# SunBangjie/FYP-BidirectionalPathTracer

Hardware: AMD Instinct MI355X
Metric: Mrays/s + RMSE vs the scalar oracle, BDPT pass, Sponza-class scene 1920x1080 depth 8 (higher is better)
Workload: dtype f32

## Files before the change

fyp-bidirectionalpathtracer_amd/csrc/api.cpp:

```cpp
#include <hip/hip_runtime.h>

#include <cmath>
#include <cstdio>
#include <cstdlib>
#include <cstring>
#include <future>
#include <functional>
#include <atomic>
#include <chrono>
#include <string>
#include <thread>
#include <vector>

#include "../../include/bdpt.h"
#include <new>

#include "bvh.h"
#include "kernels.h"
#include "refit.h"
#include "scene_bvh.h"

using namespace bdpt;

namespace {
// ... 8 lines not shown

struct bdpt_ctx {
  int device = 0;
  int numCUs = 256;
  std::string err;
  bool haveScene = false, haveCamera = false, haveSize = false;
  SceneDev S{};
  std::vector<void*> sceneAllocs;
  bdpt_bvh_info bvhInfo{};
  bdpt_camera cam{};
  bdpt_environment env{};
  uint32_t W = 0, H = 0, maxDepth = 0;
  std::vector<std::pair<uint32_t, uint32_t>> rowRanges;
  uint32_t tileRows = 0;
  SplatLayout sl{1, 1, 0};
  bdpt_stripes stripes{0, 1, 0};
  PathBuf P{};
  std::vector<void*> frameAllocs;
  unsigned long long* splat = nullptr;
  unsigned long long* ownSplat = nullptr;
  DevCounters* counters = nullptr;
  hipStream_t lastStream = nullptr;
  bool timing = false;
  hipEvent_t ev[kMaxStages + 1]{};
  const char* stageNames[kMaxStages]{};
  int numStages = 0;
  bool evCreated = false;
  static constexpr int kMaxSideStages = 4;
  hipEvent_t sideEv[2 * kMaxSideStages]{};
  const char* sideNames[kMaxSideStages]{};
  int numSideStages = 0;
  int lazyRounds = 3;
  LaunchGrids grids{};
  int* stackOvf = nullptr;
  uint32_t stackOvfStride = 0;
  unsigned long long* rayCursor = nullptr;
  unsigned long long* adaptiveSum = nullptr;
  bdpt_gbuffer ownGb{};
  float4* bmfrPos[2] = {nullptr, nullptr};
  float4* bmfrNorm[2] = {nullptr, nullptr};
  float4* bmfrNoisy[2] = {nullptr, nullptr};
  float4* bmfrFiltered[2] = {nullptr, nullptr};
  uint8_t* bmfrAccept = nullptr;
  uint32_t* bmfrPrevPixel = nullptr;
  int bmfrRead = 0;
  hipStream_t walkStream = nullptr;
  hipEvent_t evFork = nullptr, evJoin = nullptr, evSplat = nullptr;
  uint32_t* hintPix = nullptr;
  bool hints = true;
  bdpt_camera hintCam{};
  bool hintCamValid = false;
  uint32_t numVertices = 0, numTriangles = 0;
  uint32_t* lightMaps = nullptr;
  bool refitReady = false;
  BvhRefitPlan refitPlan;
  RefitDev refit{};
  uint32_t numUpdates = 0;
  float* stage[3] = {nullptr, nullptr, nullptr};
  void* pinned = nullptr;
  size_t pinnedBytes = 0;
  hipEvent_t evStage = nullptr, evOrder = nullptr;
  bool stageInFlight = false;
  unsigned long long* groupSplat = nullptr;
  uint8_t* groupLightIdx = nullptr;
};

namespace {

template <class F>
void hostParallelFor(size_t n, const F& f) {
  const int threads = bvhBuildThreads();
  if (threads <= 1 || n < 65536) {
    f((size_t)0, n);
    return;
  }
  WorkerScope pool;
  const size_t chunk = (n + (size_t)threads - 1) / (size_t)threads;
  for (int t = 1; t < threads; t++) {
    const size_t a = std::min(n, chunk * (size_t)t), b = std::min(n, a + chunk);
    if (a < b) pool.spawn([&f, a, b] { f(a, b); });
  }
  f((size_t)0, std::min(n, chunk));
  pool.join();
}

bool fail(bdpt_ctx* c, const std::string& m) {
  if (c) c->err = m;
  return false;
}
#define HIPCHK(ctx, expr)                                                                       \
  do {                                                                                          \
    hipError_t e_ = (expr);                                                                     \
    if (e_ != hipSuccess) {                                                                     \
      fail(ctx, std::string(#expr) + ": " + hipGetErrorString(e_));                             \
      return BDPT_E_HIP;                                                                        \
    }                                                                                           \
  } while (0)

template <class T>
int devAlloc(bdpt_ctx* c, std::vector<void*>& pool, T** out, size_t count) {
  void* p = nullptr;
  size_t bytes = std::max<size_t>(count * sizeof(T), 16);
  hipError_t e = hipMalloc(&p, bytes);
  if (e != hipSuccess) {
    fail(c, std::string("hipMalloc(") + std::to_string(bytes) + "): " + hipGetErrorString(e));
    return BDPT_E_NOMEM;
  }
  pool.push_back(p);
  *out = reinterpret_cast<T*>(p);
  return BDPT_OK;
}
template <class T>
int devUpload(bdpt_ctx* c, std::vector<void*>& pool, const T** out, const T* host, size_t count) {
  T* d = nullptr;
  int rc = devAlloc(c, pool, &d, count);
  if (rc) return rc;
  if (count) {
    std::string e;
    if (!bvhUploadStaged(d, host, count * sizeof(T), e)) {
      fail(c, e);
      return BDPT_E_HIP;
    }
  }
  *out = d;
  return BDPT_OK;
}
void freePool(std::vector<void*>& pool) {
  for (void* p : pool) (void)hipFree(p);
  pool.clear();
}
void freeLightGroups(bdpt_ctx* c) {
  if (c->groupSplat) (void)hipFree(c->groupSplat);
  if (c->groupLightIdx) (void)hipFree(c->groupLightIdx);
  c->groupSplat = nullptr;
  c->groupLightIdx = nullptr;
}

#define ENTER(ctx) HIPCHK(ctx, hipSetDevice((ctx)->device))

bool streamIsCapturing(hipStream_t st) {
  hipStreamCaptureStatus cs = hipStreamCaptureStatusNone;
  if (hipStreamIsCapturing(st, &cs) != hipSuccess) return false;
  return cs != hipStreamCaptureStatusNone;
}

int allocOwnGbuffer(bdpt_ctx* c) {
  if (c->ownGb.worldPosition) return BDPT_OK;
  const size_t n = (size_t)c->W * c->H;
  const size_t mark = c->frameAllocs.size();
  bdpt_gbuffer g{};
  int rc;
  if ((rc = devAlloc(c, c->frameAllocs, &g.worldPosition, n * 4)) || (rc = devAlloc(c, c->frameAllocs, &g.worldNormal, n * 4)) ||
      (rc = devAlloc(c, c->frameAllocs, &g.materialDiffuse, n * 4)) || (rc = devAlloc(c, c->frameAllocs, &g.materialSpecRough, n * 4)) ||
      (rc = devAlloc(c, c->frameAllocs, &g.materialExtraParams, n * 4)) || (rc = devAlloc(c, c->frameAllocs, &g.emissive, n * 4))) {
    while (c->frameAllocs.size() > mark) {
      (void)hipFree(c->frameAllocs.back());
      c->frameAllocs.pop_back();
    }
    return rc;
  }
  c->ownGb = g;
  return BDPT_OK;
}

int allocBmfrHistory(bdpt_ctx* c) {
  if (c->bmfrAccept) return BDPT_OK;
// ... 252 lines not shown
    std::future<SideUploads>& f;
    ~SideJoin() {
      if (!f.valid()) return;
      try {
        SideUploads u = f.get();
        for (void* q : u.pool) (void)hipFree(q);
      } catch (...) {
      }
    }
  } sideJoin{side};
  SceneBvh sb;
  try {
    std::string treeError;
    struct Build {
      BvhDeviceBuild* b;
      ~Build() { bvhDeviceBuildEnd(b); }
    } build{bvhDeviceBuildBegin(c->device, std::getenv("BDPT_HOST_COLLAPSE") == nullptr)};
    buildSceneBvh(d, 0, -1.0f, -1.0f, std::getenv("BDPT_NO_ALPHA_CLASSIFY") == nullptr, sb, buildBinaryTreeOnDevice, build.b, &treeError, packOnDevice, makeReferencesOnDevice,
                  std::getenv("BDPT_HOST_COLLAPSE") == nullptr, std::getenv("BDPT_HOST_PRIORITIES") == nullptr);
    if (sb.bvh.deviceRecs) c->sceneAllocs.push_back(sb.bvh.deviceRecs);
    if (!treeError.empty()) {
      fail(c, "scene: " + treeError);
      return treeError.find("2^31") != std::string::npos ? BDPT_E_LIMIT : (treeError.find("out of device memory") != std::string::npos ? BDPT_E_NOMEM : BDPT_E_HIP);
    }
  } catch (const std::bad_alloc&) {
    fail(c, "scene: out of host memory while building the acceleration structure");
    return BDPT_E_NOMEM;
  }
  lap("buildSceneBvh");
  Bvh& bvh = sb.bvh;
  const std::vector<uint32_t>& alphaTris = sb.alphaTris;
  if (bvh.maxStack > (uint32_t)kBvhMaxStack) {
    fail(c, "bvh needs a deeper traversal stack than the device provides");
    return BDPT_E_LIMIT;
  }
  if (!bvh.deviceRecs && !bvh.recs.empty()) {
    const BvhRec* dRecs = nullptr;
    if (int rc0 = devUpload(c, c->sceneAllocs, &dRecs, bvh.recs.data(), bvh.recs.size())) return rc0;
    bvh.deviceRecs = const_cast<BvhRec*>(dRecs);
    bvh.deviceNumRecs = bvh.recs.size();
  }
  if (!bvh.deviceRecs) {
    fail(c, "scene: the acceleration structure has no records");
    return BDPT_E_HIP;
  }
  c->bvhInfo.numNodes = bvh.numNodes;
  c->bvhInfo.numTriangles = d->numTriangles;
  c->bvhInfo.maxDepth = bvh.maxDepth;
  c->bvhInfo.nodeBytes = sizeof(BvhRec);
  c->bvhInfo.triBytes = sizeof(BvhTri);
  c->bvhInfo.sahCost = bvh.sahCost;
  c->bvhInfo.maxStack = bvh.maxStack;
  c->bvhInfo.numReferences = bvh.numRefs;
  c->bvhInfo.numDropped = bvh.numDropped;
  c->bvhInfo.numAlphaMode = sb.numAlphaMode;
  c->bvhInfo.numAlwaysPass = sb.numAlwaysPass;

  int rc;
  {
    SideUploads u = side.get();
    c->sceneAllocs.insert(c->sceneAllocs.end(), u.pool.begin(), u.pool.end());
    if (u.err != hipSuccess) {
      fail(c, std::string("scene upload: ") + (u.what.empty() ? std::string(hipGetErrorString(u.err)) : u.what));
      return u.err == hipErrorOutOfMemory ? BDPT_E_NOMEM : BDPT_E_HIP;
    }
    c->S.shade = reinterpret_cast<const float4*>(u.shade);
    c->S.indices = u.indices;
    if (d->bitangents) {
      c->S.bitangents = u.bitangents;
      c->S.hasBitangents = 1;
    }
  }
  lap("shading records + uploads (joined)");
  c->S.recs = reinterpret_cast<const uint4*>(bvh.deviceRecs);
  c->S.numRecs = (uint32_t)bvh.deviceNumRecs;
  if ((rc = devUpload(c, c->sceneAllocs, &c->S.materials, d->materials, d->numMaterials))) return rc;
  std::vector<TexDev> texs(d->numTextures);
  for (uint32_t i = 0; i < d->numTextures; i++) {
    const bdpt_texture& t = d->textures[i];
    if (!t.rgba8 || !t.width || !t.height) {
      fail(c, "scene: empty texture");
      return BDPT_E_INVALID;
    }
    const uint8_t* px;
    if ((rc = devUpload(c, c->sceneAllocs, &px, t.rgba8, (size_t)t.width * t.height * 4))) return rc;
    texs[i] = TexDev{px, t.width, t.height, t.srgb, 0};
  }
  if ((rc = devUpload(c, c->sceneAllocs, &c->S.textures, texs.data(), texs.size()))) return rc;
  {
    std::vector<TexDev> matTex((size_t)d->numMaterials * 4, TexDev{nullptr, 0, 0, 0, 0});
    for (uint32_t mi = 0; mi < d->numMaterials; mi++) {
      const bdpt_material& mm = d->materials[mi];
      const int ids[4] = {mm.texBaseColor, mm.texSpecular, mm.texEmissive, mm.texNormal};
      for (int k = 0; k < 4; k++)
        if (ids[k] >= 0) matTex[(size_t)mi * 4 + k] = texs[(size_t)ids[k]];
    }
    if ((rc = devUpload(c, c->sceneAllocs, &c->S.matTex, matTex.data(), matTex.size()))) return rc;
  }
  {
    float4* dAlpha = nullptr;
    if ((rc = devAlloc(c, c->sceneAllocs, &dAlpha, std::max<size_t>(alphaTris.size(), 1) * 4))) return rc;
    if (alphaTris.empty()) {
      HIPCHK(c, hipMemset(dAlpha, 0, 4 * sizeof(float4)));
    } else {
      const uint32_t* dList = nullptr;
      std::vector<void*> scratch;
      if ((rc = devUpload(c, scratch, &dList, alphaTris.data(), alphaTris.size()))) {
        freePool(scratch);
        return rc;
      }
      launchAlphaRecs(c->S, dList, (uint32_t)alphaTris.size(), dAlpha, nullptr);
      const hipError_t e = hipDeviceSynchronize();
      freePool(scratch);
      HIPCHK(c, e);
    }
    c->S.alphaRecs = dAlpha;
  }
  lap("indices, textures, alpha");
  SceneConst sc;
  std::memset(&sc, 0, sizeof(sc));
  std::memcpy(sc.lights, d->lights, sizeof(bdpt_light) * d->numLights);
  for (int i = 0; i < 256; i++) {
    double cc = (double)i / 255.0;
    double l = (cc <= 0.04045) ? cc / 12.92 : std::pow((cc + 0.055) / 1.055, 2.4);
    sc.srgbLut[i] = (float)l;
  }
  if ((rc = devUpload(c, c->sceneAllocs, &c->S.sc, &sc, 1))) return rc;
  c->S.numLights = d->numLights;
  c->hints = std::getenv("BDPT_NO_HINTS") == nullptr;
  if (c->hints) {
    uint32_t res = 512;
    if (const char* e = std::getenv("BDPT_LIGHT_MAP_RES")) res = (uint32_t)std::max(0, std::min(2048, std::atoi(e)));
    if (res) {
      uint32_t* maps = nullptr;
      if ((rc = devAlloc(c, c->sceneAllocs, &maps, (size_t)6 * res * res * d->numLights))) return rc;
      launchLightMaps(c->S, maps, res, nullptr);
      HIPCHK(c, hipDeviceSynchronize());
      c->S.lightMap = maps;
      c->S.lightMapRes = res;
      c->lightMaps = maps;
    }
  }
  if (c->hintPix) HIPCHK(c, hipMemset(c->hintPix, 0xFF, (size_t)c->W * c->H * sizeof(uint32_t)));
  c->hintCamValid = false;
  lap("light maps");
  c->numVertices = d->numVertices;
  c->numTriangles = d->numTriangles;
  c->haveScene = true;
  return BDPT_OK;
}
int bdpt_set_scene(bdpt_ctx* c, const bdpt_scene_desc* d) {
  try {
    return setSceneImpl(c, d);
  } catch (const std::bad_alloc&) {
    fail(c, "scene: out of host memory while building the acceleration structure");
    return BDPT_E_NOMEM;
  } catch (const std::exception& e) {
    fail(c, std::string("scene: ") + e.what());
    return BDPT_E_INVALID;
  }
}


int bdpt_get_bvh_info(const bdpt_ctx* c, bdpt_bvh_info* out) {
  if (!c || !out) return BDPT_E_INVALID;
  if (!c->haveScene) return BDPT_E_STATE;
  *out = c->bvhInfo;
  return BDPT_OK;
}

int bdpt_set_camera(bdpt_ctx* c, const bdpt_camera* cam) {
  if (!c || !cam) return BDPT_E_INVALID;
  c->cam = *cam;
  c->haveCamera = true;
  return BDPT_OK;
}

int bdpt_set_environment(bdpt_ctx* c, const bdpt_environment* env) {
  if (!c) return BDPT_E_INVALID;
  if (env && env->envMap && (!env->width || !env->height)) {
    fail(c, "environment: a map needs a width and a height");
    return BDPT_E_INVALID;
  }
  c->env = env ? *env : bdpt_environment{};
  if (!c->env.envMap) c->env.width = c->env.height = 0;
  return BDPT_OK;
}

namespace {
int ensureRefit(bdpt_ctx* c, hipStream_t st) {
  if (c->refitReady) return BDPT_OK;
  if (streamIsCapturing(st)) {
    fail(c, "update: the first update needs bdpt_prepare(BDPT_PREPARE_REFIT) before stream capture");
    return BDPT_E_STATE;
// ... 1252 lines not shown
```

fyp-bidirectionalpathtracer_amd/csrc/device_scene.hpp:

```cpp
#pragma once
#include "device_math.hpp"
#include "kernels.h"

namespace bdpt {
#define BD __device__ __forceinline__

struct f4 {
  float x, y, z, w;
};
BD f4 lerp4(f4 a, f4 b, float s) {
  return f4{a.x + (b.x - a.x) * s, a.y + (b.y - a.y) * s, a.z + (b.z - a.z) * s, a.w + (b.w - a.w) * s};
}
BD int wrapi(int i, int n) {
  int m = i % n;
  return (m < 0) ? m + n : m;
}
BD f4 texel(const SceneDev& S, const TexDev& t, int ix, int iy) {
  const uchar4 p = *reinterpret_cast<const uchar4*>(t.px + ((size_t)iy * t.w + (size_t)ix) * 4);
  f4 r;
  if (t.srgb) {
    r.x = S.sc->srgbLut[p.x];
    r.y = S.sc->srgbLut[p.y];
    r.z = S.sc->srgbLut[p.z];
  } else {
    r.x = (float)p.x / 255.0f;
    r.y = (float)p.y / 255.0f;
    r.z = (float)p.z / 255.0f;
  }
  r.w = (float)p.w / 255.0f;
  return r;
}
BD f4 sampleBilinearT(const SceneDev& S, const TexDev& t, float u, float v) {
  float x = u * (float)t.w - 0.5f;
  float y = v * (float)t.h - 0.5f;
  float x0 = floorf(x), y0 = floorf(y);
  float fx = x - x0, fy = y - y0;
  int ix0 = wrapi((int)x0, (int)t.w), iy0 = wrapi((int)y0, (int)t.h);
  int ix1 = wrapi(ix0 + 1, (int)t.w), iy1 = wrapi(iy0 + 1, (int)t.h);
  f4 t00 = texel(S, t, ix0, iy0), t10 = texel(S, t, ix1, iy0);
  f4 t01 = texel(S, t, ix0, iy1), t11 = texel(S, t, ix1, iy1);
  return lerp4(lerp4(t00, t10, fx), lerp4(t01, t11, fx), fy);
}
BD f4 sampleBilinear(const SceneDev& S, int texId, float u, float v) { return sampleBilinearT(S, S.textures[texId], u, v); }
BD f4 sampleTexture(const SceneDev& S, int texId, float u, float v, f4 factor, uint32_t mode) {
  if (mode == BDPT_CHANNEL_UNUSED) return f4{0, 0, 0, 0};
  if (mode == BDPT_CHANNEL_CONST || texId < 0) return factor;
  return sampleBilinear(S, texId, u, v);
}
BD f4 sampleTextureT(const SceneDev& S, const TexDev& t, int texId, float u, float v, f4 factor, uint32_t mode) {
  if (mode == BDPT_CHANNEL_UNUSED) return f4{0, 0, 0, 0};
  if (mode == BDPT_CHANNEL_CONST || texId < 0) return factor;
  return sampleBilinearT(S, t, u, v);
}

struct MatDev {
  f4 baseColor, specular;
  f3 emissive;
  float alphaThreshold, IoR;
  uint32_t flags;
  int texBase, texSpec, texEmis, texNorm;
};
BD MatDev loadMaterial(const SceneDev& S, uint32_t id) {
  const float4* m = reinterpret_cast<const float4*>(S.materials + id);
  float4 a = m[0], b = m[1], c = m[2], d = m[3];
  MatDev r;
  r.baseColor = f4{a.x, a.y, a.z, a.w};
  r.specular = f4{b.x, b.y, b.z, b.w};
  r.emissive = mk(c.x, c.y, c.z);
  r.alphaThreshold = c.w;
  r.IoR = d.x;
  r.flags = __float_as_uint(d.y);
  uint32_t t0 = __float_as_uint(d.z), t1 = __float_as_uint(d.w);
  r.texBase = (int)(int16_t)(t0 & 0xffffu);
  r.texSpec = (int)(int16_t)(t0 >> 16);
  r.texEmis = (int)(int16_t)(t1 & 0xffffu);
  r.texNorm = (int)(int16_t)(t1 >> 16);
  return r;
}

BD bool alphaTestFails(const SceneDev& S, uint32_t rec, float bu, float bv) {
  const float4* r = S.alphaRecs + (size_t)rec * 4;
  const float4 a0 = r[0], a1 = r[1], a2 = r[2], a3 = r[3];
  const uint32_t mode = __float_as_uint(a2.x);
  float alpha = 0.0f;
  if (mode == 1u) {
    alpha = a1.w;
  } else if (mode == 2u) {
    float u = 0, v = 0;
    const float b0 = 1.0f - bu - bv;
    u += a0.x * b0;
    v += a0.y * b0;
    u += a0.z * bu;
    v += a0.w * bu;
    u += a1.x * bv;
    v += a1.y * bv;
    const int tw = (int)__float_as_uint(a2.y), th = (int)__float_as_uint(a2.z);
    const uint8_t* px = reinterpret_cast<const uint8_t*>(((unsigned long long)__float_as_uint(a3.y) << 32) | (unsigned long long)__float_as_uint(a3.x));
    const float x = u * (float)tw - 0.5f, y = v * (float)th - 0.5f;
    const float x0 = floorf(x), y0 = floorf(y);
    const float fx = x - x0, fy = y - y0;
    const int ix0 = wrapi((int)x0, tw), iy0 = wrapi((int)y0, th);
    const int ix1 = wrapi(ix0 + 1, tw), iy1 = wrapi(iy0 + 1, th);
    const float t00 = (float)px[((size_t)iy0 * tw + (size_t)ix0) * 4 + 3] / 255.0f, t10 = (float)px[((size_t)iy0 * tw + (size_t)ix1) * 4 + 3] / 255.0f;
    const float t01 = (float)px[((size_t)iy1 * tw + (size_t)ix0) * 4 + 3] / 255.0f, t11 = (float)px[((size_t)iy1 * tw + (size_t)ix1) * 4 + 3] / 255.0f;
    const float top = t00 + (t10 - t00) * fx, bot = t01 + (t11 - t01) * fx;
    alpha = top + (bot - top) * fy;
  }
  return alpha < a1.z;
}

struct AlphaIn {
  float4 a0, a1, a2, a3;
};
BD void alphaTexels(const AlphaIn& r, float bu, float bv, bool run, float& fx, float& fy, float& t00, float& t10, float& t01, float& t11) {
  fx = fy = t00 = t10 = t01 = t11 = 0.0f;
  if (!run || __float_as_uint(r.a2.x) != 2u) return;
  float u = 0, v = 0;
  const float b0 = 1.0f - bu - bv;
  u += r.a0.x * b0;
  v += r.a0.y * b0;
  u += r.a0.z * bu;
  v += r.a0.w * bu;
  u += r.a1.x * bv;
  v += r.a1.y * bv;
  const int tw = (int)__float_as_uint(r.a2.y), th = (int)__float_as_uint(r.a2.z);
  const uint8_t* px = reinterpret_cast<const uint8_t*>(((unsigned long long)__float_as_uint(r.a3.y) << 32) | (unsigned long long)__float_as_uint(r.a3.x));
  const float x = u * (float)tw - 0.5f, y = v * (float)th - 0.5f;
  const float x0 = floorf(x), y0 = floorf(y);
  fx = x - x0;
  fy = y - y0;
  const int ix0 = wrapi((int)x0, tw), iy0 = wrapi((int)y0, th);
  const int ix1 = wrapi(ix0 + 1, tw), iy1 = wrapi(iy0 + 1, th);
  t00 = (float)px[((size_t)iy0 * tw + (size_t)ix0) * 4 + 3];
  t10 = (float)px[((size_t)iy0 * tw + (size_t)ix1) * 4 + 3];
  t01 = (float)px[((size_t)iy1 * tw + (size_t)ix0) * 4 + 3];
  t11 = (float)px[((size_t)iy1 * tw + (size_t)ix1) * 4 + 3];
}
BD bool alphaVerdict(const AlphaIn& r, float fx, float fy, float t00, float t10, float t01, float t11) {
  const uint32_t mode = __float_as_uint(r.a2.x);
  float alpha = 0.0f;
  if (mode == 1u) {
    alpha = r.a1.w;
  } else if (mode == 2u) {
    const float w00 = t00 / 255.0f, w10 = t10 / 255.0f, w01 = t01 / 255.0f, w11 = t11 / 255.0f;
    const float top = w00 + (w10 - w00) * fx, bot = w01 + (w11 - w01) * fx;
    alpha = top + (bot - top) * fy;
  }
  return alpha < r.a1.z;
}
BD void alphaTestFails2(const SceneDev& S, bool need0, uint32_t rec0, float u0, float v0, bool need1, uint32_t rec1, float u1, float v1,
                        bool& fail0, bool& fail1) {
  AlphaIn r0, r1;
  r0.a0 = r0.a1 = r0.a2 = r0.a3 = r1.a0 = r1.a1 = r1.a2 = r1.a3 = make_float4(0.0f, 0.0f, 0.0f, 0.0f);
  if (need0) {
    const float4* p = S.alphaRecs + (size_t)rec0 * 4;
    r0.a0 = p[0];
    r0.a1 = p[1];
    r0.a2 = p[2];
    r0.a3 = p[3];
  }
  if (need1) {
    const float4* p = S.alphaRecs + (size_t)rec1 * 4;
    r1.a0 = p[0];
    r1.a1 = p[1];
    r1.a2 = p[2];
    r1.a3 = p[3];
  }
  float fx0, fy0, a00, a10, a01, a11, fx1, fy1, b00, b10, b01, b11;
  alphaTexels(r0, u0, v0, need0, fx0, fy0, a00, a10, a01, a11);
  alphaTexels(r1, u1, v1, need1, fx1, fy1, b00, b10, b01, b11);
  fail0 = need0 && alphaVerdict(r0, fx0, fy0, a00, a10, a01, a11);
  fail1 = need1 && alphaVerdict(r1, fx1, fy1, b00, b10, b01, b11);
}

struct Shading {
  f3 posW, V, N, diffuse, specular, emissive;
  float opacity, linearRoughness, roughness, IoR;
};
template <bool NMAP>
BD Shading shadeHit(const SceneDev& S, uint32_t prim, float bu, float bv, f3 camPosW) {
  const float4* r = S.shade + (size_t)prim * kShadeRecF4;
  const float4 r0 = r[0], r1 = r[1], r2 = r[2], r3 = r[3], r4 = r[4], r5 = r[5], r6 = r[6];
  const float b0 = 1.0f - bu - bv;
  float u = 0, v = 0;
  f3 normalW = mk(0), posW = mk(0);
  u += r1.z * b0;
  v += r1.w * b0;
  normalW = normalW + mk(r0.w, r1.x, r1.y) * b0;
  posW = posW + mk(r0.x, r0.y, r0.z) * b0;
  u += r3.z * bu;
  v += r3.w * bu;
  normalW = normalW + mk(r2.w, r3.x, r3.y) * bu;
  posW = posW + mk(r2.x, r2.y, r2.z) * bu;
  u += r5.z * bv;
  v += r5.w * bv;
  normalW = normalW + mk(r4.w, r5.x, r5.y) * bv;
  posW = posW + mk(r4.x, r4.y, r4.z) * bv;
  normalW = normalize(normalW);

  const uint32_t matId = __float_as_uint(r6.x);
  const MatDev m = loadMaterial(S, matId);
  const TexDev tBase = S.matTex[(size_t)matId * 4], tSpec = S.matTex[(size_t)matId * 4 + 1], tEmis = S.matTex[(size_t)matId * 4 + 2];
  Shading sd;
  f4 base = sampleTextureT(S, tBase, m.texBase, u, v, m.baseColor, BDPT_FLAG_DIFFUSE_TYPE(m.flags));
  sd.opacity = m.baseColor.w;
  sd.posW = posW;
  sd.V = normalize(camPosW - posW);
  sd.N = normalize(normalW);
  f4 spec = sampleTextureT(S, tSpec, m.texSpec, u, v, m.specular, BDPT_FLAG_SPECULAR_TYPE(m.flags));
  f3 baseRgb = mk(base.x, base.y, base.z);
  if (BDPT_FLAG_SHADING_MODEL(m.flags) == BDPT_SHADING_MODEL_METAL_ROUGH) {
    sd.diffuse = lerp3(baseRgb, mk(0), spec.z);
    sd.specular = lerp3(mk(0.04f), baseRgb, spec.z);
    sd.linearRoughness = spec.y;
  } else {
    sd.diffuse = baseRgb;
    sd.specular = mk(spec.x, spec.y, spec.z);
    sd.linearRoughness = 1.0f - spec.w;
  }
// ... 40 lines not shown
```

fyp-bidirectionalpathtracer_amd/csrc/kernels.h:

```cpp
#pragma once
#include <hip/hip_runtime.h>
#include <stdint.h>

#include "../../include/bdpt.h"

namespace bdpt {

constexpr int kWave = 64;
#ifndef KSTACK
#define KSTACK 32
#endif
constexpr int kStackEntries = KSTACK;
#ifndef BDPT_STACK_LDS
#define BDPT_STACK_LDS 24
#endif
constexpr int kStackLds = BDPT_STACK_LDS < KSTACK ? BDPT_STACK_LDS : KSTACK;
constexpr int kMaxPersistentPerCU = 32;
constexpr int kStackOvfRows = KSTACK - kStackLds;
constexpr int kShadeRecF4 = 7;
constexpr uint32_t kNoRay = 0xFFFFFFFFu;
constexpr uint32_t kNumSubQueues = 32;
#ifndef BDPT_FETCH_CHUNK
#define BDPT_FETCH_CHUNK 256
#endif
constexpr uint32_t kFetchChunk = BDPT_FETCH_CHUNK;
constexpr uint32_t kCursorStride = 32;
constexpr uint32_t kCursorBlock = kNumSubQueues * kCursorStride;
#ifndef BDPT_RAY_SUBQUEUES
#define BDPT_RAY_SUBQUEUES 32
#endif
constexpr uint32_t kNumRaySubQueues = BDPT_RAY_SUBQUEUES;
constexpr uint32_t kRayCursorBlock = kNumRaySubQueues * kCursorStride;
constexpr uint32_t kCounterShards = 64;

enum : int { F_COL = 0, F_POS = 3, F_N = 6, F_V = 9, F_DIF = 12, F_SPEC = 15, F_ROUGH = 18, F_ISSPEC = 19, F_PDF = 20, NF = 21 };
constexpr int NF4 = 6;
enum : int { PATH_EYE = 0, PATH_LIGHT = 1 };
enum : int { RAY_TERMS = 0, RAY_PAIRS = 1 };

struct TexDev {
  const uint8_t* px;
  uint32_t w, h, srgb, pad;
};

struct SceneConst {
  bdpt_light lights[BDPT_MAX_LIGHTS];
  float srgbLut[256];
};

struct SceneDev {
  const uint4* recs;
  const float4* shade;
  const float* bitangents;
  const uint32_t* indices;
  const bdpt_material* materials;
  const TexDev* textures;
  const TexDev* matTex;
  const SceneConst* sc;
  uint32_t numLights;
  uint32_t hasBitangents;
  uint32_t numRecs;
  const float4* alphaRecs;
  int* stackOvf;
  uint32_t stackOvfStride;
  const uint32_t* lightMap;
  uint32_t lightMapRes;
};

struct DevCounters {
  unsigned long long v[kCounterShards][32];
};
enum : int {
  C_RAYS_PRIMARY = 0, C_RAYS_EYE, C_RAYS_LIGHT, C_RAYS_NEE, C_RAYS_SPLAT, C_RAYS_CONNECT,
  C_NODE_CLOSEST, C_TRI_CLOSEST, C_NODE_SHADOW, C_TRI_SHADOW, C_PIX_VALID, C_SPLATS, C_RAYS_LAZY,
  C_STACK_MAX,
  C_ALPHA_CLOSEST, C_ALPHA_SHADOW,
  C_HINT_NEE, C_HINT_SPLAT
};

inline __host__ __device__ uint32_t numConnectPairs(uint32_t D) {
  uint32_t n = 0;
  for (uint32_t t = 2; t <= D; t++) n += (t < D - 1) ? t : (D - 1);
  return n;
}

struct PathBuf {
  float* v;
  float* rayDir;
  const uint32_t* pix;
  uint32_t* seedE;
  uint32_t* seedL;
  uint8_t* eyeLast;
  uint8_t* lightLast;
  uint8_t* lightReal;
  uint32_t* queue[3];
  uint32_t pathSubCap;
  uint32_t* qcount;
  uint32_t* qhead;
  float* rayQ;
  float* rayContrib;
  uint8_t* rayVis;
  uint32_t* rayCount;
  uint32_t* rayHead;
  uint32_t raySubCap[2];
  uint32_t rayBase[2];
  uint32_t* slotRay;
  uint32_t* splatPix;
  float* misE;
  float* misL;
  uint8_t* lazyCursor;
  uint32_t* lazyRay;
  uint32_t* lazyCount;
  uint32_t rayCap;
  uint32_t Np, D1;
};

struct SplatLayout {
  uint32_t stripeRows, owners, chunkRows;
};
inline __host__ __device__ size_t splatIndex(const SplatLayout& L, uint32_t W, uint32_t x, uint32_t y) {
  const uint32_t s = y / L.stripeRows;
  const uint32_t owner = s % L.owners, row = (s / L.owners) * L.stripeRows + (y - s * L.stripeRows);
  return ((size_t)owner * L.chunkRows + row) * W + x;
}

struct FrameDev {
  bdpt_camera cam;
  bdpt_params p;
  uint32_t W, H;
  SplatLayout sl;
  float* out;
  unsigned long long* splat;
  bdpt_gbuffer gb;
  DevCounters* counters;
  const float* envMap;
  uint32_t envW, envH;
  float envColor[3];
  const uint32_t* hintPix;
};

struct GroupDev {
  float* planes;
  unsigned long long* splat;
  uint8_t* lightIdx;
  uint32_t numLights;
  uint64_t framePix;
};

struct MaskDev {
  const uint8_t* mask;
  uint32_t* eye;
  uint32_t* eyeCount;
  const uint32_t* walkEye;
  const uint32_t* walkEyeCount;
};

enum class FrameKind { Plain, Groups, Masked };
struct FrameVariant {
  FrameKind kind = FrameKind::Plain;
  GroupDev groups{};
  MaskDev mask{};
};

struct GBufferDev {
  bdpt_camera cam;
  bdpt_gbuffer_params gp;
  uint32_t W, H, Np;
  const uint32_t* pix;
  bdpt_gbuffer gb;
  DevCounters* counters;
  uint32_t* hintPix;
};

struct BmfrDev {
  uint32_t W, H, frame;
  uint32_t full, doPre;
  float m[16];
  const float4* curPos;
  const uint16_t* curNorm;
  const uint16_t* albedo;
  float4* noisy;
  const float4 *prevPosR, *prevNormR, *prevNoisyR, *prevFilteredR;
  float4 *prevPosW, *prevNormW, *prevNoisyW, *prevFilteredW;
  uint8_t* accept;
  uint32_t* prevPixel;
};
void launchBmfr(const BmfrDev& A, uint32_t flags, hipStream_t st);

void launchGBuffer(const SceneDev& S, const GBufferDev& G, hipStream_t st);
void launchAlphaRecs(const SceneDev& S, const uint32_t* alphaTris, uint32_t n, float4* out, hipStream_t st);
void launchHintFill(const SceneDev& S, const GBufferDev& G, hipStream_t st);
void launchLightMaps(const SceneDev& S, uint32_t* maps, uint32_t res, hipStream_t st);
void launchInitPaths(const SceneDev& S, const FrameDev& F, const PathBuf& P, const FrameVariant& V, hipStream_t st);
struct LaunchGrids {
  uint32_t walk[16] = {};
  uint32_t shadow[2] = {0, 0};
  uint32_t rays[3] = {0, 0, 0};
};
void launchWalk(const SceneDev& S, const FrameDev& F, const PathBuf& P, const FrameVariant& V, LaunchGrids& G, int numCUs,
                hipStream_t st);
void launchMisPrefix(const FrameDev& F, const PathBuf& P, hipStream_t st);
void launchGenNee(const SceneDev& S, const FrameDev& F, const PathBuf& P, hipStream_t st);
void launchGenSplat(const SceneDev& S, const FrameDev& F, const PathBuf& P, hipStream_t st);
void launchGenConnect(const SceneDev& S, const FrameDev& F, const PathBuf& P, hipStream_t st);
void launchTraceShadow(const SceneDev& S, const FrameDev& F, const PathBuf& P, int rayClass, LaunchGrids& G, int numCUs, hipStream_t st);
void launchTraceRays(const SceneDev& S, const float4* rays, uint32_t cap, const uint32_t* count, unsigned long long* cursor, int mode,
                     float4* hits, uint8_t* vis, LaunchGrids& G, int numCUs, hipStream_t st);
void launchGather(const FrameDev& F, const PathBuf& P, const FrameVariant& V, uint32_t* lazyList, uint32_t* lazyCount, hipStream_t st);
void launchLazyGen(const FrameDev& F, const PathBuf& P, const uint32_t* list, const uint32_t* listCount, int batch, hipStream_t st);
void launchLazyCheck(const FrameDev& F, const PathBuf& P, const FrameVariant& V, const uint32_t* list, const uint32_t* listCount,
                     int batch, uint32_t* nextList, uint32_t* nextCount, hipStream_t st);
constexpr int kLazyBatchDiv = 8;
constexpr int kMaxLazyRounds = 8;
void launchResolve(const unsigned long long* splat, bool tileLocal, uint32_t splatRow0, const SplatLayout& L, float* out, uint32_t W,
                   const uint32_t* pix, uint32_t Np, hipStream_t st);
void launchFrameResolve(const FrameDev& F, const PathBuf& P, const FrameVariant& V, hipStream_t st);
struct AdaptiveDev {
  float4* mean;
  float* m2;
  uint32_t* count;
  uint8_t* mask;
  uint32_t* active;
  float4* frame;
  uint32_t W, H;
  float threshold, epsilon;
  uint32_t minSamples, maxSamples, blockSize;
};
void launchAdaptiveUpdate(const AdaptiveDev& A, unsigned long long* scratch, hipStream_t st);
void launchAdaptiveReset(const AdaptiveDev& A, hipStream_t st);
void launchAccumulate(float* last, float* cur, uint32_t accumCount, uint32_t maxAccum, uint64_t numTexels, hipStream_t st);
void launchAccumulateTile(float* last, float* cur, uint32_t accumCount, uint32_t maxAccum, const uint32_t* pix, uint32_t Np,
                          hipStream_t st);
void launchTilePack(const void* frame, void* packed, uint32_t bytesPerPixel, const uint32_t* pix, uint32_t Np, hipStream_t st);
void launchTileUnpack(const void* packed, void* frame, uint32_t bytesPerPixel, uint32_t W, uint32_t H, uint32_t stripeRows, uint32_t owners,
                      uint32_t owner, uint32_t packedRows, hipStream_t st);
void launchTestRng(const uint32_t* v0, const uint32_t* v1, uint32_t n, uint32_t draws, uint32_t* states, float* floats,
                   hipStream_t st);
void launchTestTrace(const SceneDev& S, const float* rays, uint32_t n, int mode, int32_t* prim, float* tuv, hipStream_t st);
void launchTestTraceShadow(const SceneDev& S, const float* planes, uint32_t cap, const uint32_t* count, uint32_t* head, uint8_t* vis,
                           DevCounters* counters, float tmin, int numCUs, hipStream_t st);
void launchTestBsdf(const float* in, uint32_t n, uint32_t matIndex, float* out, hipStream_t st);

}
```

fyp-bidirectionalpathtracer_amd/csrc/kernels.hip:

```cpp
#include "kernels.h"

#include <algorithm>
#include <type_traits>

#include "device_math.hpp"
#include "device_scene.hpp"
#include "device_trace.hpp"
#include "launch.hpp"

namespace bdpt {

#define BD __device__ __forceinline__

BD void wavePush(bool active, uint32_t value, uint32_t* items, uint32_t* count, uint32_t subCap, uint32_t q = 0xffffffffu) {
  unsigned long long mask = __ballot(active);
  if (mask == 0ull) return;
  const int lane = (int)(threadIdx.x & 63u);
  const int leader = __ffsll((long long)mask) - 1;
  if (q == 0xffffffffu) q = blockIdx.x % kNumSubQueues;
  uint32_t base = 0;
  if (lane == leader) base = atomicAdd(&count[q * kCursorStride], (uint32_t)__popcll(mask));
  base = (uint32_t)__shfl((int)base, leader);
  const uint32_t prefix = (uint32_t)__popcll(mask & ((1ull << lane) - 1ull));
  if (active) items[q * subCap + base + prefix] = value;
// ... 1389 lines not shown
  const float* r = rays + (size_t)i * 8;
  uint32_t a = 0, b = 0;
  Hit h = traverse<MODE, false>(S, ld3(r), ld3(r + 3), r[6], r[7], s_stack + threadIdx.x, a, b);
  if (MODE != 2 && h.prim >= 0) {
    const bool named = h.rec < S.numRecs && (int)__float_as_uint(reinterpret_cast<const float4*>(S.recs)[(size_t)h.rec * kRecF4].w) == h.prim;
    if (!named) h.prim = -2;
  }
  prim[i] = h.prim;
  const bool rec = (MODE != 2) && h.prim >= 0;
  tuv[(size_t)i * 3] = rec ? h.t : 0.0f;
  tuv[(size_t)i * 3 + 1] = rec ? h.u : 0.0f;
  tuv[(size_t)i * 3 + 2] = rec ? h.v : 0.0f;
}
template <bool GGX>
__global__ void test_bsdf_kernel(const float* in, uint32_t n, bool fromLobe, float* out) {
  const uint32_t i = blockIdx.x * blockDim.x + threadIdx.x;
  if (i >= n) return;
  const float* p = in + (size_t)i * 20;
  f3 N = ld3(p), V = ld3(p + 3), Lq = ld3(p + 6), dif = ld3(p + 9), spec = ld3(p + 12);
  float rough = p[15];
  bool isSpec = p[16] != 0.0f;
  uint32_t seed = __float_as_uint(p[17]);
  f3 L;
  float pdf;
  bool sSpec;
  f3 w = sampleBRDF<GGX>(seed, N, N, V, dif, spec, rough, fromLobe, L, pdf, sSpec);
  f3 fr = evalBRDF<GGX>(V, Lq, N, N, dif, spec, rough, isSpec);
  float* o = out + (size_t)i * 16;
  o[0] = w.x;
  o[1] = w.y;
  o[2] = w.z;
  o[3] = L.x;
  o[4] = L.y;
  o[5] = L.z;
  o[6] = pdf;
  o[7] = sSpec ? 1.0f : 0.0f;
  o[8] = fr.x;
  o[9] = fr.y;
  o[10] = fr.z;
  o[11] = o[12] = o[13] = o[14] = o[15] = 0.0f;
}


static inline uint32_t blocksFor(uint64_t n) { return (uint32_t)((n + kWave - 1) / kWave); }
static inline uint32_t queueGrid(const PathBuf& P) { return (P.pathSubCap / kWave) * kNumSubQueues; }


template <class Fn>
static void withFlags(Fn&& fn) {
  fn();
}
template <class Fn, class... Flags>
static void withFlags(Fn&& fn, bool f, Flags... rest) {
  if (f)
    withFlags([&](auto... t) { fn(std::true_type{}, t...); }, rest...);
  else
    withFlags([&](auto... t) { fn(std::false_type{}, t...); }, rest...);
}
template <class Fn>
static void withKind(FrameKind kind, Fn&& fn) {
  if (kind == FrameKind::Groups)
    fn(std::integral_constant<FrameKind, FrameKind::Groups>{});
  else if (kind == FrameKind::Masked)
    fn(std::integral_constant<FrameKind, FrameKind::Masked>{});
  else
    fn(std::integral_constant<FrameKind, FrameKind::Plain>{});
}
template <FrameKind K>
static FrameArg<K> frameArg(const FrameVariant& V) {
  if constexpr (K == FrameKind::Groups)
    return V.groups;
  else if constexpr (K == FrameKind::Masked)
    return V.mask;
  else
    return NoArg{};
}

void launchGBuffer(const SceneDev& S, const GBufferDev& G, hipStream_t st) {
  const uint32_t Np = G.Np;
  if (!Np) return;
  withFlags([&](auto CNT) { launchWave(gbuffer_kernel<CNT>, blocksFor(Np), st, S, G); }, G.counters != nullptr);
}

__global__ void alpha_recs_kernel(SceneDev S, const uint32_t* __restrict__ alphaTris, uint32_t n, float4* __restrict__ out) {
  const uint32_t i = blockIdx.x * blockDim.x + threadIdx.x;
  if (i >= n) return;
  const uint32_t t = alphaTris[i];
  const float4* sr = S.shade + (size_t)t * kShadeRecF4;
  const float4 a1 = sr[1], b1 = sr[3], c1 = sr[5], m6 = sr[6];
  const uint32_t mid = __float_as_uint(m6.x);
  const bdpt_material& m = S.materials[mid];
  const uint32_t type = BDPT_FLAG_DIFFUSE_TYPE(m.flags);
  uint32_t mode = 0, tw = 0, th = 0;
  unsigned long long px = 0;
  if (type == BDPT_CHANNEL_UNUSED) {
    mode = 0;
  } else if (type == BDPT_CHANNEL_CONST || m.texBaseColor < 0) {
    mode = 1;
  } else {
    mode = 2;
    const TexDev td = S.matTex[(size_t)mid * 4];
    tw = td.w;
    th = td.h;
    px = (unsigned long long)reinterpret_cast<uintptr_t>(td.px);
  }
  float4* r = out + (size_t)i * 4;
  r[0] = make_float4(a1.z, a1.w, b1.z, b1.w);
  r[1] = make_float4(c1.z, c1.w, m.alphaThreshold, m.baseColor[3]);
  r[2] = make_float4(__uint_as_float(mode), __uint_as_float(tw), __uint_as_float(th), 0.0f);
  r[3] = make_float4(__uint_as_float((uint32_t)(px & 0xffffffffull)), __uint_as_float((uint32_t)(px >> 32)), 0.0f, 0.0f);
}
void launchAlphaRecs(const SceneDev& S, const uint32_t* alphaTris, uint32_t n, float4* out, hipStream_t st) {
  if (!n) return;
  hipLaunchKernelGGL(alpha_recs_kernel, dim3((n + 255) / 256), dim3(256), 0, st, S, alphaTris, n, out);
}

void launchHintFill(const SceneDev& S, const GBufferDev& G, hipStream_t st) {
  if (!G.Np || !G.hintPix) return;
  launchWave(gbuffer_kernel<false, true>, (uint32_t)(blocksFor(G.Np)), st, S, G);
}

void launchLightMaps(const SceneDev& S, uint32_t* maps, uint32_t res, hipStream_t st) {
  const uint64_t n = (uint64_t)6 * res * res * S.numLights;
  if (!n) return;
  launchWave(light_map_kernel, (uint32_t)((n + kWave - 1) / kWave), st, S, maps, res);
}

void launchInitPaths(const SceneDev& S, const FrameDev& F, const PathBuf& P, const FrameVariant& V, hipStream_t st) {
  if (!P.Np) return;
  withKind(V.kind, [&](auto K) {
    withFlags([&](auto GGX) { launchWave(init_paths_kernel<GGX, K>, blocksFor(P.Np), st, S, F, P, frameArg<K>(V)); }, F.p.matIndex == 0);
  });
}

void launchWalk(const SceneDev& S, const FrameDev& F, const PathBuf& P, const FrameVariant& V, LaunchGrids& G, int numCUs,
                hipStream_t st) {
  if (!P.Np || F.p.maxDepth < 1) return;
  const bool cnt = (F.p.flags & BDPT_PARAM_COUNTERS) != 0, ggx = F.p.matIndex == 0;
  const bool ext = (F.p.flags & (BDPT_PARAM_ENV_ON_MISS | BDPT_PARAM_EMISSIVE_HITS)) != 0, masked = V.kind == FrameKind::Masked;
  uint32_t& g = G.walk[(masked ? 8 : 0) + (ext ? 4 : 0) + (ggx ? 2 : 0) + (cnt ? 1 : 0)];
  const uint32_t need = blocksFor((uint64_t)2 * P.Np);
  withFlags(
      [&](auto GGX, auto CNT, auto EXT, auto MASKED) {
        const auto kernel = walk_kernel<GGX, CNT, EXT, MASKED>;
        if (!g) g = persistentGrid(kernel, numCUs);
        launchWave(kernel, std::min(g, need), st, S, F, P, P.qhead, frameArg<MASKED ? FrameKind::Masked : FrameKind::Plain>(V));
      },
      ggx, cnt, ext, masked);
}

void launchMisPrefix(const FrameDev& F, const PathBuf& P, hipStream_t st) {
  if (!P.Np) return;
  launchWave(mis_prefix_kernel, (uint32_t)(queueGrid(P)), st, F, P);
}
void launchGenNee(const SceneDev& S, const FrameDev& F, const PathBuf& P, hipStream_t st) {
  if (!P.Np) return;
  withFlags([&](auto GGX, auto WIDE) { launchWave(gen_nee_kernel<GGX, WIDE ? 16 : 8>, queueGrid(P) * (WIDE ? 16 : 8), st, S, F, P); },
            F.p.matIndex == 0, P.D1 > 9);
}
void launchGenSplat(const SceneDev& S, const FrameDev& F, const PathBuf& P, hipStream_t st) {
  if (!P.Np || (F.p.flags & BDPT_PARAM_NO_SPLAT)) return;
  withFlags([&](auto GGX, auto WIDE) { launchWave(gen_splat_kernel<GGX, WIDE ? 16 : 8>, queueGrid(P) * (WIDE ? 16 : 8), st, S, F, P); },
            F.p.matIndex == 0, P.D1 > 9);
}
void launchGenConnect(const SceneDev& S, const FrameDev& F, const PathBuf& P, hipStream_t st) {
  if (!P.Np || (F.p.flags & BDPT_PARAM_NO_CONNECT) || F.p.maxDepth < 2) return;
  withFlags([&](auto GGX, auto WIDE) { launchWave(gen_connect_kernel<GGX, WIDE ? 16 : 8>, queueGrid(P) * (WIDE ? 16 : 8), st, S, F, P); },
            F.p.matIndex == 0, P.D1 > 9);
}

void launchTraceShadow(const SceneDev& S, const FrameDev& F, const PathBuf& P, int cls, LaunchGrids& G, int numCUs, hipStream_t st) {
  if (!P.Np) return;
  const bool cnt = (F.p.flags & BDPT_PARAM_COUNTERS) != 0;
  RayQueue Q{P.rayQ + P.rayBase[cls], P.rayCap, P.raySubCap[cls], kNumRaySubQueues, P.rayCount + (size_t)cls * kRayCursorBlock,
             P.rayHead + (size_t)cls * kRayCursorBlock};
  uint8_t* vis = P.rayVis + P.rayBase[cls];
  uint32_t& g = G.shadow[cnt ? 1 : 0];
  withFlags(
      [&](auto CNT) {
        if (!g) g = persistentGrid(trace_shadow_kernel<CNT>, numCUs);
        launchWave(trace_shadow_kernel<CNT>, g, st, S, Q, vis, F.counters, F.p.minT);
      },
      cnt);
}

void launchGather(const FrameDev& F, const PathBuf& P, const FrameVariant& V, uint32_t* lazyList, uint32_t* lazyCount, hipStream_t st) {
  if (!P.Np) return;
  withKind(V.kind, [&](auto K) { launchWave(gather_kernel<K>, queueGrid(P), st, F, P, lazyList, lazyCount, frameArg<K>(V)); });
}
void launchLazyGen(const FrameDev& F, const PathBuf& P, const uint32_t* list, const uint32_t* listCount, int batch, hipStream_t st) {
  if (!P.Np) return;
  withFlags([&](auto WIDE) { launchWave(lazy_gen_kernel<WIDE ? 16 : 8>, queueGrid(P) * (WIDE ? 16 : 8), st, F, P, list, listCount, batch); },
            P.D1 > 9);
}
void launchLazyCheck(const FrameDev& F, const PathBuf& P, const FrameVariant& V, const uint32_t* list, const uint32_t* listCount,
                     int batch, uint32_t* nextList, uint32_t* nextCount, hipStream_t st) {
  if (!P.Np) return;
// ... 104 lines not shown
```

Before: 4727.

## Pack alpha bilinear quads into per-texture planes and merge texel row loads

At scene load, builds a per-texture plane in which each texel stores the four neighbouring alpha bytes of its bilinear footprint. Alpha tests in traversal then do a single 32-bit load instead of four scattered byte loads. Bilinear texture sampling now fetches each row pair with one 64-bit load and uses power-of-two masking for wrap instead of modulo; textures are padded by 4 bytes so the wide load stays in bounds. The cost is extra device memory and host preprocessing for alpha textures.

```diff
diff --git a/fyp-bidirectionalpathtracer_amd/csrc/api.cpp b/fyp-bidirectionalpathtracer_amd/csrc/api.cpp
--- a/fyp-bidirectionalpathtracer_amd/csrc/api.cpp
+++ b/fyp-bidirectionalpathtracer_amd/csrc/api.cpp
@@ -114,6 +114,12 @@
   }
   f((size_t)0, std::min(n, chunk));
   pool.join();
+}
+
+std::vector<uint32_t> alphaQuadPlane(const bdpt_texture& t) {
+  std::vector<uint32_t> q((size_t)t.width * t.height);
+  hostParallelFor(t.height, [&](size_t y0, size_t y1) { alphaQuadRows(t.rgba8, t.width, t.height, (uint32_t)y0, (uint32_t)y1, q.data()); });
+  return q;
 }
 
 bool fail(bdpt_ctx* c, const std::string& m) {
@@ -532,9 +538,18 @@
       fail(c, "scene: empty texture");
       return BDPT_E_INVALID;
     }
-    const uint8_t* px;
-    if ((rc = devUpload(c, c->sceneAllocs, &px, t.rgba8, (size_t)t.width * t.height * 4))) return rc;
-    texs[i] = TexDev{px, t.width, t.height, t.srgb, 0};
+    const size_t bytes = (size_t)t.width * t.height * 4;
+    uint8_t* px = nullptr;
+    if ((rc = devAlloc(c, c->sceneAllocs, &px, bytes + 4))) return rc;
+    HIPCHK(c, hipMemset(px + bytes, 0, 4));
+    {
+      std::string e;
+      if (!bvhUploadStaged(px, t.rgba8, bytes, e)) {
+        fail(c, e);
+        return BDPT_E_HIP;
+      }
+    }
+    texs[i] = TexDev{px, t.width, t.height, t.srgb, texPow2Flags(t.width, t.height)};
   }
   if ((rc = devUpload(c, c->sceneAllocs, &c->S.textures, texs.data(), texs.size()))) return rc;
   {
@@ -553,13 +568,27 @@
     if (alphaTris.empty()) {
       HIPCHK(c, hipMemset(dAlpha, 0, 4 * sizeof(float4)));
     } else {
+      std::vector<uint8_t> alphaMat(d->numMaterials, 0);
+      for (const uint32_t t : alphaTris) alphaMat[d->triMaterial[t]] = 1;
+      std::vector<unsigned long long> quadByTex(std::max<size_t>(d->numTextures, 1), 0ull);
+      for (uint32_t mi = 0; mi < d->numMaterials; mi++) {
+        const bdpt_material& mm = d->materials[mi];
+        if (!alphaMat[mi] || !alphaSamplesTexture(BDPT_FLAG_DIFFUSE_TYPE(mm.flags), mm.texBaseColor) || quadByTex[(size_t)mm.texBaseColor])
+          continue;
+        const std::vector<uint32_t> plane = alphaQuadPlane(d->textures[mm.texBaseColor]);
+        const uint32_t* dPlane = nullptr;
+        if ((rc = devUpload(c, c->sceneAllocs, &dPlane, plane.data(), plane.size()))) return rc;
+        quadByTex[(size_t)mm.texBaseColor] = (unsigned long long)reinterpret_cast<uintptr_t>(dPlane);
+      }
       const uint32_t* dList = nullptr;
+      const unsigned long long* dQuad = nullptr;
       std::vector<void*> scratch;
-      if ((rc = devUpload(c, scratch, &dList, alphaTris.data(), alphaTris.size()))) {
+      if ((rc = devUpload(c, scratch, &dList, alphaTris.data(), alphaTris.size())) ||
+          (rc = devUpload(c, scratch, &dQuad, quadByTex.data(), quadByTex.size()))) {
         freePool(scratch);
         return rc;
       }
-      launchAlphaRecs(c->S, dList, (uint32_t)alphaTris.size(), dAlpha, nullptr);
+      launchAlphaRecs(c->S, dList, (uint32_t)alphaTris.size(), dQuad, dAlpha, nullptr);
       const hipError_t e = hipDeviceSynchronize();
       freePool(scratch);
       HIPCHK(c, e);
diff --git a/fyp-bidirectionalpathtracer_amd/csrc/device_scene.hpp b/fyp-bidirectionalpathtracer_amd/csrc/device_scene.hpp
--- a/fyp-bidirectionalpathtracer_amd/csrc/device_scene.hpp
+++ b/fyp-bidirectionalpathtracer_amd/csrc/device_scene.hpp
@@ -11,23 +11,27 @@
 BD f4 lerp4(f4 a, f4 b, float s) {
   return f4{a.x + (b.x - a.x) * s, a.y + (b.y - a.y) * s, a.z + (b.z - a.z) * s, a.w + (b.w - a.w) * s};
 }
-BD int wrapi(int i, int n) {
-  int m = i % n;
-  return (m < 0) ? m + n : m;
-}
-BD f4 texel(const SceneDev& S, const TexDev& t, int ix, int iy) {
-  const uchar4 p = *reinterpret_cast<const uchar4*>(t.px + ((size_t)iy * t.w + (size_t)ix) * 4);
+typedef __attribute__((address_space(1))) const uint32_t gU32;
+typedef __attribute__((address_space(1), aligned(4))) const unsigned long long gU64a4;
+BD void texelRow(const uint8_t* px, uint32_t w, int iy, int ix0, int ix1, uint32_t& a, uint32_t& b) {
+  gU32* row = (gU32*)px + (size_t)iy * w;
+  const unsigned long long q = *(gU64a4*)(row + ix0);
+  a = (uint32_t)q;
+  b = (uint32_t)(q >> 32);
+  if (ix1 != ix0 + 1) b = row[ix1];
+}
+BD f4 texel(const SceneDev& S, const TexDev& t, uint32_t p) {
   f4 r;
   if (t.srgb) {
-    r.x = S.sc->srgbLut[p.x];
-    r.y = S.sc->srgbLut[p.y];
-    r.z = S.sc->srgbLut[p.z];
+    r.x = S.sc->srgbLut[p & 0xffu];
+    r.y = S.sc->srgbLut[(p >> 8) & 0xffu];
+    r.z = S.sc->srgbLut[(p >> 16) & 0xffu];
   } else {
-    r.x = (float)p.x / 255.0f;
-    r.y = (float)p.y / 255.0f;
-    r.z = (float)p.z / 255.0f;
-  }
-  r.w = (float)p.w / 255.0f;
+    r.x = (float)(p & 0xffu) / 255.0f;
+    r.y = (float)((p >> 8) & 0xffu) / 255.0f;
+    r.z = (float)((p >> 16) & 0xffu) / 255.0f;
+  }
+  r.w = (float)(p >> 24) / 255.0f;
   return r;
 }
 BD f4 sampleBilinearT(const SceneDev& S, const TexDev& t, float u, float v) {
@@ -35,10 +39,13 @@
   float y = v * (float)t.h - 0.5f;
   float x0 = floorf(x), y0 = floorf(y);
   float fx = x - x0, fy = y - y0;
-  int ix0 = wrapi((int)x0, (int)t.w), iy0 = wrapi((int)y0, (int)t.h);
-  int ix1 = wrapi(ix0 + 1, (int)t.w), iy1 = wrapi(iy0 + 1, (int)t.h);
-  f4 t00 = texel(S, t, ix0, iy0), t10 = texel(S, t, ix1, iy0);
-  f4 t01 = texel(S, t, ix0, iy1), t11 = texel(S, t, ix1, iy1);
+  int ix0 = wrapT((int)x0, (int)t.w, (t.pow2 & kTexPow2W) != 0u), iy0 = wrapT((int)y0, (int)t.h, (t.pow2 & kTexPow2H) != 0u);
+  int ix1 = wrapNext(ix0, (int)t.w), iy1 = wrapNext(iy0, (int)t.h);
+  uint32_t p00, p10, p01, p11;
+  texelRow(t.px, t.w, iy0, ix0, ix1, p00, p10);
+  texelRow(t.px, t.w, iy1, ix0, ix1, p01, p11);
+  f4 t00 = texel(S, t, p00), t10 = texel(S, t, p10);
+  f4 t01 = texel(S, t, p01), t11 = texel(S, t, p11);
   return lerp4(lerp4(t00, t10, fx), lerp4(t01, t11, fx), fy);
 }
 BD f4 sampleBilinear(const SceneDev& S, int texId, float u, float v) { return sampleBilinearT(S, S.textures[texId], u, v); }
@@ -78,6 +85,17 @@
   return r;
 }
 
+BD uint32_t alphaQuad(const float4& a2, const float4& a3, float u, float v, float& fx, float& fy) {
+  const int tw = (int)__float_as_uint(a2.y), th = (int)__float_as_uint(a2.z);
+  const uint32_t pow2 = __float_as_uint(a2.w);
+  gU32* px = (gU32*)(((unsigned long long)__float_as_uint(a3.y) << 32) | (unsigned long long)__float_as_uint(a3.x));
+  const float x = u * (float)tw - 0.5f, y = v * (float)th - 0.5f;
+  const float x0 = floorf(x), y0 = floorf(y);
+  fx = x - x0;
+  fy = y - y0;
+  const int ix0 = wrapT((int)x0, tw, (pow2 & kTexPow2W) != 0u), iy0 = wrapT((int)y0, th, (pow2 & kTexPow2H) != 0u);
+  return px[(size_t)iy0 * tw + (size_t)ix0];
+}
 BD bool alphaTestFails(const SceneDev& S, uint32_t rec, float bu, float bv) {
   const float4* r = S.alphaRecs + (size_t)rec * 4;
   const float4 a0 = r[0], a1 = r[1], a2 = r[2], a3 = r[3];
@@ -94,15 +112,10 @@
     v += a0.w * bu;
     u += a1.x * bv;
     v += a1.y * bv;
-    const int tw = (int)__float_as_uint(a2.y), th = (int)__float_as_uint(a2.z);
-    const uint8_t* px = reinterpret_cast<const uint8_t*>(((unsigned long long)__float_as_uint(a3.y) << 32) | (unsigned long long)__float_as_uint(a3.x));
-    const float x = u * (float)tw - 0.5f, y = v * (float)th - 0.5f;
-    const float x0 = floorf(x), y0 = floorf(y);
-    const float fx = x - x0, fy = y - y0;
-    const int ix0 = wrapi((int)x0, tw), iy0 = wrapi((int)y0, th);
-    const int ix1 = wrapi(ix0 + 1, tw), iy1 = wrapi(iy0 + 1, th);
-    const float t00 = (float)px[((size_t)iy0 * tw + (size_t)ix0) * 4 + 3] / 255.0f, t10 = (float)px[((size_t)iy0 * tw + (size_t)ix1) * 4 + 3] / 255.0f;
-    const float t01 = (float)px[((size_t)iy1 * tw + (size_t)ix0) * 4 + 3] / 255.0f, t11 = (float)px[((size_t)iy1 * tw + (size_t)ix1) * 4 + 3] / 255.0f;
+    float fx, fy;
+    const uint32_t q = alphaQuad(a2, a3, u, v, fx, fy);
+    const float t00 = (float)(q & 0xffu) / 255.0f, t10 = (float)((q >> 8) & 0xffu) / 255.0f;
+    const float t01 = (float)((q >> 16) & 0xffu) / 255.0f, t11 = (float)(q >> 24) / 255.0f;
     const float top = t00 + (t10 - t00) * fx, bot = t01 + (t11 - t01) * fx;
     alpha = top + (bot - top) * fy;
   }
@@ -123,18 +136,11 @@
   v += r.a0.w * bu;
   u += r.a1.x * bv;
   v += r.a1.y * bv;
-  const int tw = (int)__float_as_uint(r.a2.y), th = (int)__float_as_uint(r.a2.z);
-  const uint8_t* px = reinterpret_cast<const uint8_t*>(((unsigned long long)__float_as_uint(r.a3.y) << 32) | (unsigned long long)__float_as_uint(r.a3.x));
-  const float x = u * (float)tw - 0.5f, y = v * (float)th - 0.5f;
-  const float x0 = floorf(x), y0 = floorf(y);
-  fx = x - x0;
-  fy = y - y0;
-  const int ix0 = wrapi((int)x0, tw), iy0 = wrapi((int)y0, th);
-  const int ix1 = wrapi(ix0 + 1, tw), iy1 = wrapi(iy0 + 1, th);
-  t00 = (float)px[((size_t)iy0 * tw + (size_t)ix0) * 4 + 3];
-  t10 = (float)px[((size_t)iy0 * tw + (size_t)ix1) * 4 + 3];
-  t01 = (float)px[((size_t)iy1 * tw + (size_t)ix0) * 4 + 3];
-  t11 = (float)px[((size_t)iy1 * tw + (size_t)ix1) * 4 + 3];
+  const uint32_t q = alphaQuad(r.a2, r.a3, u, v, fx, fy);
+  t00 = (float)(q & 0xffu);
+  t10 = (float)((q >> 8) & 0xffu);
+  t01 = (float)((q >> 16) & 0xffu);
+  t11 = (float)(q >> 24);
 }
 BD bool alphaVerdict(const AlphaIn& r, float fx, float fy, float t00, float t10, float t01, float t11) {
   const uint32_t mode = __float_as_uint(r.a2.x);
diff --git a/fyp-bidirectionalpathtracer_amd/csrc/kernels.h b/fyp-bidirectionalpathtracer_amd/csrc/kernels.h
--- a/fyp-bidirectionalpathtracer_amd/csrc/kernels.h
+++ b/fyp-bidirectionalpathtracer_amd/csrc/kernels.h
@@ -3,6 +3,7 @@
 #include <stdint.h>
 
 #include "../../include/bdpt.h"
+#include "texture_planes.h"
 
 namespace bdpt {
 
@@ -40,7 +41,7 @@
 
 struct TexDev {
   const uint8_t* px;
-  uint32_t w, h, srgb, pad;
+  uint32_t w, h, srgb, pow2;
 };
 
 struct SceneConst {
@@ -188,7 +189,7 @@
 void launchBmfr(const BmfrDev& A, uint32_t flags, hipStream_t st);
 
 void launchGBuffer(const SceneDev& S, const GBufferDev& G, hipStream_t st);
-void launchAlphaRecs(const SceneDev& S, const uint32_t* alphaTris, uint32_t n, float4* out, hipStream_t st);
+void launchAlphaRecs(const SceneDev& S, const uint32_t* alphaTris, uint32_t n, const unsigned long long* quadByTex, float4* out, hipStream_t st);
 void launchHintFill(const SceneDev& S, const GBufferDev& G, hipStream_t st);
 void launchLightMaps(const SceneDev& S, uint32_t* maps, uint32_t res, hipStream_t st);
 void launchInitPaths(const SceneDev& S, const FrameDev& F, const PathBuf& P, const FrameVariant& V, hipStream_t st);
diff --git a/fyp-bidirectionalpathtracer_amd/csrc/kernels.hip b/fyp-bidirectionalpathtracer_amd/csrc/kernels.hip
--- a/fyp-bidirectionalpathtracer_amd/csrc/kernels.hip
+++ b/fyp-bidirectionalpathtracer_amd/csrc/kernels.hip
@@ -1495,7 +1495,8 @@
   withFlags([&](auto CNT) { launchWave(gbuffer_kernel<CNT>, blocksFor(Np), st, S, G); }, G.counters != nullptr);
 }
 
-__global__ void alpha_recs_kernel(SceneDev S, const uint32_t* __restrict__ alphaTris, uint32_t n, float4* __restrict__ out) {
+__global__ void alpha_recs_kernel(SceneDev S, const uint32_t* __restrict__ alphaTris, uint32_t n, const unsigned long long* __restrict__ quadByTex,
+                                  float4* __restrict__ out) {
   const uint32_t i = blockIdx.x * blockDim.x + threadIdx.x;
   if (i >= n) return;
   const uint32_t t = alphaTris[i];
@@ -1504,28 +1505,29 @@
   const uint32_t mid = __float_as_uint(m6.x);
   const bdpt_material& m = S.materials[mid];
   const uint32_t type = BDPT_FLAG_DIFFUSE_TYPE(m.flags);
-  uint32_t mode = 0, tw = 0, th = 0;
+  uint32_t mode = 0, tw = 0, th = 0, pow2 = 0;
   unsigned long long px = 0;
   if (type == BDPT_CHANNEL_UNUSED) {
     mode = 0;
-  } else if (type == BDPT_CHANNEL_CONST || m.texBaseColor < 0) {
+  } else if (!alphaSamplesTexture(type, m.texBaseColor)) {
     mode = 1;
   } else {
     mode = 2;
     const TexDev td = S.matTex[(size_t)mid * 4];
     tw = td.w;
     th = td.h;
-    px = (unsigned long long)reinterpret_cast<uintptr_t>(td.px);
+    pow2 = td.pow2;
+    px = quadByTex[m.texBaseColor];
   }
   float4* r = out + (size_t)i * 4;
   r[0] = make_float4(a1.z, a1.w, b1.z, b1.w);
   r[1] = make_float4(c1.z, c1.w, m.alphaThreshold, m.baseColor[3]);
-  r[2] = make_float4(__uint_as_float(mode), __uint_as_float(tw), __uint_as_float(th), 0.0f);
+  r[2] = make_float4(__uint_as_float(mode), __uint_as_float(tw), __uint_as_float(th), __uint_as_float(pow2));
   r[3] = make_float4(__uint_as_float((uint32_t)(px & 0xffffffffull)), __uint_as_float((uint32_t)(px >> 32)), 0.0f, 0.0f);
 }
-void launchAlphaRecs(const SceneDev& S, const uint32_t* alphaTris, uint32_t n, float4* out, hipStream_t st) {
+void launchAlphaRecs(const SceneDev& S, const uint32_t* alphaTris, uint32_t n, const unsigned long long* quadByTex, float4* out, hipStream_t st) {
   if (!n) return;
-  hipLaunchKernelGGL(alpha_recs_kernel, dim3((n + 255) / 256), dim3(256), 0, st, S, alphaTris, n, out);
+  hipLaunchKernelGGL(alpha_recs_kernel, dim3((n + 255) / 256), dim3(256), 0, st, S, alphaTris, n, quadByTex, out);
 }
 
 void launchHintFill(const SceneDev& S, const GBufferDev& G, hipStream_t st) {
diff --git a/fyp-bidirectionalpathtracer_amd/csrc/texture_planes.h b/fyp-bidirectionalpathtracer_amd/csrc/texture_planes.h
--- /dev/null
+++ b/fyp-bidirectionalpathtracer_amd/csrc/texture_planes.h
@@ -0,0 +1,43 @@
+#pragma once
+#include <stddef.h>
+#include <stdint.h>
+
+#include "../../include/bdpt.h"
+
+#if defined(__HIPCC__)
+#define BDPT_HD __host__ __device__ inline
+#else
+#define BDPT_HD inline
+#endif
+
+namespace bdpt {
+
+enum : uint32_t { kTexPow2W = 1u, kTexPow2H = 2u };
+BDPT_HD uint32_t texPow2Flags(uint32_t w, uint32_t h) {
+  return ((w & (w - 1u)) == 0u ? kTexPow2W : 0u) | ((h & (h - 1u)) == 0u ? kTexPow2H : 0u);
+}
+
+BDPT_HD int wrapi(int i, int n) {
+  int m = i % n;
+  return (m < 0) ? m + n : m;
+}
+BDPT_HD int wrapT(int i, int n, bool pow2) { return pow2 ? (i & (n - 1)) : wrapi(i, n); }
+BDPT_HD int wrapNext(int i, int n) { return (i + 1 == n) ? 0 : i + 1; }
+
+BDPT_HD bool alphaSamplesTexture(uint32_t diffuseType, int texBaseColor) {
+  return diffuseType != BDPT_CHANNEL_UNUSED && diffuseType != BDPT_CHANNEL_CONST && texBaseColor >= 0;
+}
+
+inline void alphaQuadRows(const uint8_t* rgba8, uint32_t w, uint32_t h, uint32_t y0, uint32_t y1, uint32_t* out) {
+  for (uint32_t y = y0; y < y1; y++) {
+    const uint32_t yn = (uint32_t)wrapNext((int)y, (int)h);
+    for (uint32_t x = 0; x < w; x++) {
+      const uint32_t xn = (uint32_t)wrapNext((int)x, (int)w);
+      const uint32_t a00 = rgba8[((size_t)y * w + x) * 4 + 3], a10 = rgba8[((size_t)y * w + xn) * 4 + 3];
+      const uint32_t a01 = rgba8[((size_t)yn * w + x) * 4 + 3], a11 = rgba8[((size_t)yn * w + xn) * 4 + 3];
+      out[(size_t)y * w + x] = a00 | (a10 << 8) | (a01 << 16) | (a11 << 24);
+    }
+  }
+}
+
+}
```

Result: faster. 4838, median of 6 (+2.4%).
